# mrafidashti/neuradar

Measured on NVIDIA B200. Metric: train_step_rays_per_sec, higher is better.
Workload: dtype f32

## Files before the change

### neuradar_b200/csrc/common.cuh

```cuda
#pragma once

#include <cuda_runtime.h>
#include <stdint.h>

#include "neuradar_b200.h"

namespace nrb {

constexpr int kWarp = 32;
constexpr unsigned kFull = 0xffffffffu;

void set_error(const char* fmt, ...);
void count_launch();
int finish_launch(const char* what);

inline bool aligned16(const void* p) { return (reinterpret_cast<uintptr_t>(p) & 15u) == 0; }

#define NRB_REQUIRE(cond, code, ...) \
  do {                               \
    if (!(cond)) {                   \
      ::nrb::set_error(__VA_ARGS__); \
      return (code);                 \
    }                                \
  } while (0)

int check_grid(const nrb_grid_t* g);
int check_rays(const nrb_rays_t* r);
int check_intervals(const char* who, const nrb_intervals_t* iv);

inline unsigned blocks_for(int64_t work, int threads) { return static_cast<unsigned>((work + threads - 1) / threads); }
int sm_count();
cudaError_t ensure_dynamic_smem(const void* kernel, int bytes);

__device__ __forceinline__ float mul(float a, float b) { return __fmul_rn(a, b); }
__device__ __forceinline__ float add(float a, float b) { return __fadd_rn(a, b); }
__device__ __forceinline__ float sub(float a, float b) { return __fsub_rn(a, b); }
__device__ __forceinline__ float div(float a, float b) { return __fdiv_rn(a, b); }

constexpr float kThird = 0.333333343267440796f;

struct Gaussian {
  float x, y, z;
  float std;
};

__device__ __forceinline__ Gaussian contract_gaussian(float mx, float my, float mz, float std, float scale) {
  mx = div(mx, scale);
  my = div(my, scale);
  mz = div(mz, scale);
  std = div(std, scale);
  const float mag = fmaxf(fmaxf(fabsf(mx), fabsf(my)), fabsf(mz));
  if (!(mag < 1.0f)) {
    const float cm = fmaxf(mag, 1.0f);
    const float k = sub(2.0f, div(1.0f, cm));
    mx = mul(k, div(mx, cm));
    my = mul(k, div(my, cm));
    mz = mul(k, div(mz, cm));
    const float r = div(powf(sub(mul(2.0f, cm), 1.0f), kThird), cm);
    std = mul(std, mul(r, r));
  }
  Gaussian g;
  g.x = mul(add(mx, 2.0f), 0.25f);
  g.y = mul(add(my, 2.0f), 0.25f);
  g.z = mul(add(mz, 2.0f), 0.25f);
  g.std = mul(std, 0.25f);
  return g;
}

__device__ __forceinline__ Gaussian world_gaussian(float ox, float oy, float oz, float dx, float dy, float dz,
                                                   float pixel_area, float start, float end) {
  const float dist = mul(sub(end, start), 0.5f);
  const float t = add(start, dist);
  Gaussian g;
  g.x = add(ox, mul(dx, t));
  g.y = add(oy, mul(dy, t));
  g.z = add(oz, mul(dz, t));
  const float area = mul(pixel_area, mul(t, t));
  g.std = powf(mul(area, dist), kThird);
  return g;
}

__device__ __forceinline__ Gaussian sample_gaussian(float ox, float oy, float oz, float dx, float dy, float dz,
                                                    float pixel_area, float start, float end, float scale) {
  const Gaussian w = world_gaussian(ox, oy, oz, dx, dy, dz, pixel_area, start, end);
  return contract_gaussian(w.x, w.y, w.z, w.std, scale);
}

__device__ __forceinline__ float level_weight(float scal, float std) {
  return div(1.0f, fmaxf(mul(mul(scal, 2.0f), std), 1.0f));
}

constexpr uint32_t kPrimeY = 2654435761u;
constexpr uint32_t kPrimeZ = 805459861u;

struct Cell {
  uint32_t row[8];
  float ox, oy, oz;
};

__device__ __forceinline__ Cell locate_cell(float px, float py, float pz, float scal, uint32_t mask) {
  const float sx = mul(px, scal), sy = mul(py, scal), sz = mul(pz, scal);
  const float fx = floorf(sx), fy = floorf(sy), fz = floorf(sz);
  Cell c;
  c.ox = sub(sx, fx);
  c.oy = sub(sy, fy);
  c.oz = sub(sz, fz);
  const uint32_t xf = static_cast<uint32_t>(static_cast<int32_t>(fx));
  const uint32_t xc = static_cast<uint32_t>(static_cast<int32_t>(ceilf(sx)));
  const uint32_t yf = static_cast<uint32_t>(static_cast<int32_t>(fy)) * kPrimeY;
  const uint32_t yc = static_cast<uint32_t>(static_cast<int32_t>(ceilf(sy))) * kPrimeY;
  const uint32_t zf = static_cast<uint32_t>(static_cast<int32_t>(fz)) * kPrimeZ;
  const uint32_t zc = static_cast<uint32_t>(static_cast<int32_t>(ceilf(sz))) * kPrimeZ;
  c.row[0] = (xc ^ yc ^ zc) & mask;
  c.row[1] = (xc ^ yf ^ zc) & mask;
  c.row[2] = (xf ^ yf ^ zc) & mask;
  c.row[3] = (xf ^ yc ^ zc) & mask;
  c.row[4] = (xc ^ yc ^ zf) & mask;
  c.row[5] = (xc ^ yf ^ zf) & mask;
  c.row[6] = (xf ^ yf ^ zf) & mask;
  c.row[7] = (xf ^ yc ^ zf) & mask;
  return c;
}

__device__ __forceinline__ void corner_weights(const Cell& c, float w[8]) {
  const float ax = c.ox, bx = 1.0f - c.ox, ay = c.oy, by = 1.0f - c.oy, az = c.oz, bz = 1.0f - c.oz;
  w[0] = ax * ay * az;
  w[1] = ax * by * az;
  w[2] = bx * by * az;
  w[3] = bx * ay * az;
  w[4] = ax * ay * bz;
  w[5] = ax * by * bz;
  w[6] = bx * by * bz;
  w[7] = bx * ay * bz;
}

template <int F>
struct Feat;
template <>
struct Feat<1> {
  using type = float;
};
template <>
struct Feat<2> {
  using type = float2;
};
template <>
struct Feat<4> {
  using type = float4;
};

template <int F>
__device__ __forceinline__ void load_row(const float* __restrict__ base, uint32_t row, float v[F]) {
  using V = typename Feat<F>::type;
  const V t = __ldg(reinterpret_cast<const V*>(base) + row);
  if constexpr (F == 1) {
    v[0] = t;
  } else if constexpr (F == 2) {
    v[0] = t.x;
    v[1] = t.y;
  } else {
    v[0] = t.x;
    v[1] = t.y;
    v[2] = t.z;
    v[3] = t.w;
  }
}

template <int F>
__device__ __forceinline__ void load_x_pair(const float* __restrict__ base, uint32_t row_f, uint32_t row_c, float vf[F],
                                            float vc[F]) {
  if constexpr (F == 1) {
    if (row_c == (row_f ^ 1u)) {
      const bool f_low = (row_f & 1u) == 0;
      const float2 t = __ldg(reinterpret_cast<const float2*>(base) + (row_f >> 1));
      vf[0] = f_low ? t.x : t.y;
      vc[0] = f_low ? t.y : t.x;
      return;
    }
  }
  load_row<F>(base, row_f, vf);
  load_row<F>(base, row_c, vc);
}

template <int F>
__device__ __forceinline__ void interpolate(const float* __restrict__ level_base, const Cell& c, float out[F]) {
  float f[8][F];
  load_x_pair<F>(level_base, c.row[3], c.row[0], f[3], f[0]);
  load_x_pair<F>(level_base, c.row[2], c.row[1], f[2], f[1]);
  load_x_pair<F>(level_base, c.row[7], c.row[4], f[7], f[4]);
  load_x_pair<F>(level_base, c.row[6], c.row[5], f[6], f[5]);
  const float ax = c.ox, bx = 1.0f - c.ox, ay = c.oy, by = 1.0f - c.oy, az = c.oz, bz = 1.0f - c.oz;
#pragma unroll
  for (int j = 0; j < F; ++j) {
    const float f03 = f[0][j] * ax + f[3][j] * bx;
    const float f12 = f[1][j] * ax + f[2][j] * bx;
    const float f56 = f[5][j] * ax + f[6][j] * bx;
    const float f47 = f[4][j] * ax + f[7][j] * bx;
    const float f0312 = f03 * ay + f12 * by;
    const float f4756 = f47 * ay + f56 * by;
    out[j] = f0312 * az + f4756 * bz;
  }
}

template <int F>
__device__ __forceinline__ float3 position_grad(const float* __restrict__ level_base, const Cell& c, const float (&g)[F]) {
  float f[8][F];
#pragma unroll
  for (int k = 0; k < 8; ++k) load_row<F>(level_base, c.row[k], f[k]);
  const float ax = c.ox, bx = 1.0f - c.ox, ay = c.oy, by = 1.0f - c.oy, az = c.oz, bz = 1.0f - c.oz;
  float gx = 0.f, gy = 0.f, gz = 0.f;
#pragma unroll
  for (int j = 0; j < F; ++j) {
    const float f03 = f[0][j] * ax + f[3][j] * bx, f12 = f[1][j] * ax + f[2][j] * bx;
    const float f56 = f[5][j] * ax + f[6][j] * bx, f47 = f[4][j] * ax + f[7][j] * bx;
    const float f0312 = f03 * ay + f12 * by, f4756 = f47 * ay + f56 * by;
    gz += g[j] * (f0312 - f4756);
    gy += g[j] * ((f03 - f12) * az + (f47 - f56) * bz);
    gx += g[j] * (((f[0][j] - f[3][j]) * ay + (f[1][j] - f[2][j]) * by) * az +
                  ((f[4][j] - f[7][j]) * ay + (f[5][j] - f[6][j]) * by) * bz);
  }
  return make_float3(gx, gy, gz);
}

__device__ __forceinline__ const float* tile_image_chunk(const float* img, int64_t m, int c) {
  return img + ((m >> 7) * 1024 + (m & 127)) * 4 + c * 512;
}

__device__ __forceinline__ float warp_sum(float v) {
#pragma unroll
  for (int o = 16; o > 0; o >>= 1) v += __shfl_xor_sync(kFull, v, o);
  return v;
}

__device__ __forceinline__ float warp_inclusive_sum(float v, int lane) {
#pragma unroll
  for (int o = 1; o < 32; o <<= 1) {
    const float n = __shfl_up_sync(kFull, v, o);
    if (lane >= o) v += n;
  }
  return v;
}

__device__ __forceinline__ double warp_inclusive_sum(double v, int lane) {
#pragma unroll
  for (int o = 1; o < 32; o <<= 1) {
    const double n = __shfl_up_sync(kFull, v, o);
    if (lane >= o) v += n;
  }
  return v;
}

__device__ __forceinline__ float warp_inclusive_prod(float v, int lane) {
#pragma unroll
  for (int o = 1; o < 32; o <<= 1) {
    const float n = __shfl_up_sync(kFull, v, o);
    if (lane >= o) v *= n;
  }
  return v;
}

__device__ __forceinline__ float nan_to_num(float v) {
  if (isnan(v)) return 0.0f;
  if (isinf(v)) return v > 0 ? 3.402823466e+38f : -3.402823466e+38f;
  return v;
}

__device__ __forceinline__ float power_fn(float x, float lam) {
  const float lam1 = fabsf(lam - 1.0f);
  const float base = add(div(x, lam1), 1.0f);
  const float p = (lam == -1.0f) ? div(1.0f, base) : powf(base, lam);
  return mul(div(lam1, lam), sub(p, 1.0f));
}

// ... 14 lines not shown
```

### neuradar_b200/csrc/hash_bwd_plan.cuh

```cuda
#pragma once

#include <algorithm>

#include "common.cuh"

namespace nrb {

struct GridDev {
  const float* table;
  float scalings[NRB_MAX_LEVELS];
  int num_levels;
  int log2_size;
};

inline GridDev to_dev(const nrb_grid_t* g) {
  GridDev d;
  d.table = g->table;
  for (int i = 0; i < NRB_MAX_LEVELS; ++i) d.scalings[i] = g->scalings[i];
  d.num_levels = g->num_levels;
  d.log2_size = g->log2_hashmap_size;
  return d;
}

struct BwdPlan {
  float* scratch;
  int64_t offset[NRB_MAX_LEVELS];
  int64_t stride[NRB_MAX_LEVELS];
  int copies[NRB_MAX_LEVELS];
  int r1[NRB_MAX_LEVELS];
};

template <int F>
__device__ __forceinline__ void scatter_row(float* __restrict__ base, uint32_t row, const float (&v)[F]) {
  float* p = base + static_cast<size_t>(row) * F;
  if constexpr (F == 1) {
    atomicAdd(p, v[0]);
  } else if constexpr (F == 2) {
    atomicAdd(reinterpret_cast<float2*>(p), make_float2(v[0], v[1]));
  } else {
    atomicAdd(reinterpret_cast<float4*>(p), make_float4(v[0], v[1], v[2], v[3]));
  }
}

template <int F>
__device__ __forceinline__ void scatter_x_pair(float* __restrict__ base, uint32_t row_f, uint32_t row_c,
                                               const float (&vf)[F], const float (&vc)[F], bool quad) {
  if (row_c == row_f) {
    float t[F];
#pragma unroll
    for (int j = 0; j < F; ++j) t[j] = vf[j] + vc[j];
    scatter_row<F>(base, row_f, t);
    return;
  }
  if constexpr (F == 1) {
    if (quad && (row_f ^ row_c) < 4u) {
      const uint32_t sf = row_f & 3u, sc = row_c & 3u;
      const float4 t = make_float4(sf == 0 ? vf[0] : (sc == 0 ? vc[0] : 0.0f), sf == 1 ? vf[0] : (sc == 1 ? vc[0] : 0.0f),
                                   sf == 2 ? vf[0] : (sc == 2 ? vc[0] : 0.0f), sf == 3 ? vf[0] : (sc == 3 ? vc[0] : 0.0f));
      atomicAdd(reinterpret_cast<float4*>(base) + (row_f >> 2), t);
      return;
    }
  } else if constexpr (F == 2) {
    if (row_c == (row_f ^ 1u)) {
      const bool f_low = (row_f & 1u) == 0;
      atomicAdd(reinterpret_cast<float4*>(base) + (row_f >> 1), f_low ? make_float4(vf[0], vf[1], vc[0], vc[1])
                                                                     : make_float4(vc[0], vc[1], vf[0], vf[1]));
      return;
    }
  }
  scatter_row<F>(base, row_f, vf);
  scatter_row<F>(base, row_c, vc);
}

template <int F>
__device__ __forceinline__ void scatter_rows8(float* __restrict__ base, const uint32_t (&row)[8], const float (&v)[8][F],
                                              bool quad) {
  scatter_x_pair<F>(base, row[3], row[0], v[3], v[0], quad);
  scatter_x_pair<F>(base, row[2], row[1], v[2], v[1], quad);
  scatter_x_pair<F>(base, row[7], row[4], v[7], v[4], quad);
  scatter_x_pair<F>(base, row[6], row[5], v[6], v[5], quad);
}

template <int F>
__device__ __forceinline__ void scatter_corners(const BwdPlan& plan, int l, int log2_size, int xf, int yf, int zf, int xc,
                                                int yc, int zc, const uint32_t (&hashed_rows)[8], const float (&v)[8][F],
                                                float* __restrict__ dtable, unsigned spread) {
  const int copies = plan.copies[l];
  if (copies > 1) {
    const int R1 = plan.r1[l];
    if (xf >= 0 && yf >= 0 && zf >= 0 && xc < R1 && yc < R1 && zc < R1) {
      float* rep = plan.scratch + plan.offset[l] + static_cast<size_t>(spread % static_cast<unsigned>(copies)) * plan.stride[l];
      const int cx[8] = {xc, xc, xf, xf, xc, xc, xf, xf};
      const int cy[8] = {yc, yf, yf, yc, yc, yf, yf, yc};
      const int cz[8] = {zc, zc, zc, zc, zf, zf, zf, zf};
      uint32_t rows[8];
#pragma unroll
      for (int k = 0; k < 8; ++k) rows[k] = static_cast<uint32_t>((cz[k] * R1 + cy[k]) * R1 + cx[k]);
      scatter_rows8<F>(rep, rows, v, true);
      return;
    }
  }
  scatter_rows8<F>(dtable + (static_cast<size_t>(l) << log2_size) * F, hashed_rows, v, log2_size >= 2);
}

constexpr int kMergeMaxRuns = 26;

template <int F>
__device__ __forceinline__ void merge_runs_and_scatter(const BwdPlan& plan, int l, int log2_size, float px, float py,
                                                       float pz, float scal, const Cell& c, float (&v)[8][F], bool valid,
                                                       int lane, float* __restrict__ dtable, unsigned spread) {
  const float sx = mul(px, scal), sy = mul(py, scal), sz = mul(pz, scal);
  const int xf = static_cast<int>(floorf(sx)), yf = static_cast<int>(floorf(sy)), zf = static_cast<int>(floorf(sz));
  const int xc = static_cast<int>(ceilf(sx)), yc = static_cast<int>(ceilf(sy)), zc = static_cast<int>(ceilf(sz));
  const int ceq = (xc == xf ? 1 : 0) | (yc == yf ? 2 : 0) | (zc == zf ? 4 : 0) | (valid ? 8 : 0);
  const int pxf = __shfl_up_sync(kFull, xf, 1), pyf = __shfl_up_sync(kFull, yf, 1), pzf = __shfl_up_sync(kFull, zf, 1);
  const int pce = __shfl_up_sync(kFull, ceq, 1);
  const bool head = lane == 0 || pxf != xf || pyf != yf || pzf != zf || pce != ceq;
  const unsigned heads = __ballot_sync(kFull, head);
  bool issue = valid;
  if (__popc(heads) <= kMergeMaxRuns) {
    const unsigned above = heads & ~((2u << lane) - 1u);
    const int next_head = above != 0 ? __ffs(above) - 1 : 32;
#pragma unroll
    for (int d = 1; d < 32; d <<= 1) {
      const bool take = lane + d < next_head;
      if (!__any_sync(kFull, take)) break;
#pragma unroll
      for (int k = 0; k < 8; ++k)
#pragma unroll
        for (int j = 0; j < F; ++j) {
          const float t = __shfl_down_sync(kFull, v[k][j], d);
          if (take) v[k][j] += t;
        }
    }
    issue = valid && head;
  }
  if (issue) scatter_corners<F>(plan, l, log2_size, xf, yf, zf, xc, yc, zc, c.row, v, dtable, spread);
}

inline int64_t plan_hash_bwd(const nrb_grid_t* grid, int64_t M, BwdPlan* plan) {
  constexpr double kMaxBytesPerLevel = 32.0 * 1024 * 1024;
  const int F = grid->features_per_level;
  const double table_rows = static_cast<double>(int64_t{1} << grid->log2_hashmap_size);
  int64_t floats = 0;
  for (int l = 0; l < NRB_MAX_LEVELS; ++l) {
    plan->copies[l] = 0;
    plan->offset[l] = 0;
    plan->stride[l] = 0;
    plan->r1[l] = 0;
    if (l >= grid->num_levels || M < (int64_t{1} << 16)) continue;
    const int64_t r1 = static_cast<int64_t>(grid->scalings[l]) + 1;
    const double verts = static_cast<double>(r1) * r1 * r1;
    if (verts * 1.5 > table_rows || r1 > 1024) continue;
    const int64_t per_copy = (r1 * r1 * r1 * F + 3) & ~int64_t{3};
    int copies = std::min(static_cast<int>(table_rows / verts + 0.5), 1024);
    while (copies > 1 && static_cast<double>(copies) * per_copy * 4 > kMaxBytesPerLevel) --copies;
    if (copies <= 1) continue;
    plan->copies[l] = copies;
    plan->stride[l] = per_copy;
    plan->offset[l] = floats;
    plan->r1[l] = static_cast<int>(r1);
    floats += static_cast<int64_t>(copies) * per_copy;
    floats = (floats + 3) & ~int64_t{3};
  }
  return floats * 4;
}

inline int prepare_bwd_plan(const nrb_grid_t* grid, int64_t M, void* workspace, int64_t workspace_bytes, cudaStream_t s,
                            BwdPlan* plan, int64_t* vertices) {
  const int64_t need = plan_hash_bwd(grid, M, plan);
  *vertices = 0;
  if (need > 0 && workspace != nullptr && workspace_bytes >= need && aligned16(workspace)) {
    plan->scratch = static_cast<float*>(workspace);
    cudaError_t e = cudaMemsetAsync(workspace, 0, static_cast<size_t>(need), s);
    NRB_REQUIRE(e == cudaSuccess, static_cast<int>(e), "backward workspace memset failed: %s", cudaGetErrorString(e));
    for (int l = 0; l < grid->num_levels; ++l)
      if (plan->copies[l] > 1) *vertices += static_cast<int64_t>(plan->r1[l]) * plan->r1[l] * plan->r1[l];
  } else {
    plan->scratch = nullptr;
    for (int l = 0; l < NRB_MAX_LEVELS; ++l) plan->copies[l] = 0;
  }
  return NRB_OK;
}

void launch_fold(const nrb_grid_t* grid, const BwdPlan& plan, float* dtable, int64_t vertices, cudaStream_t s);

}
```

### neuradar_b200/csrc/hash_grid.cu

```cuda
#include <algorithm>
#include <cstdlib>

#include "common.cuh"
#include "hash_bwd_plan.cuh"

namespace nrb {

template <int F>
__global__ void __launch_bounds__(256) hash_fwd_kernel(const __grid_constant__ GridDev g, const float* __restrict__ x,
                                                       const float* __restrict__ std, float* __restrict__ out,
                                                       int64_t total) {
  const int64_t gid = static_cast<int64_t>(blockIdx.x) * blockDim.x + threadIdx.x;
  if (gid >= total) return;
  const int64_t m = gid / g.num_levels;
  const int l = static_cast<int>(gid - m * g.num_levels);
  const float scal = g.scalings[l];
  const Cell c = locate_cell(__ldg(x + 3 * m), __ldg(x + 3 * m + 1), __ldg(x + 3 * m + 2), scal,
                             (1u << g.log2_size) - 1u);
  const float* base = g.table + (static_cast<size_t>(l) << g.log2_size) * F;
  float v[F];
  interpolate<F>(base, c, v);
  if (std != nullptr) {
    const float w = level_weight(scal, __ldg(std + m));
#pragma unroll
    for (int j = 0; j < F; ++j) v[j] *= w;
  }
  using V = typename Feat<F>::type;
  V o;
  if constexpr (F == 1) {
    o = v[0];
  } else if constexpr (F == 2) {
    o = make_float2(v[0], v[1]);
  } else {
    o = make_float4(v[0], v[1], v[2], v[3]);
  }
  reinterpret_cast<V*>(out)[gid] = o;
}

constexpr int kFwdWarps = 8;

template <int F>
__global__ void __launch_bounds__(kFwdWarps * 32) hash_fwd_rows_kernel(const __grid_constant__ GridDev g,
                                                                      const float* __restrict__ x,
                                                                      const float* __restrict__ std,
                                                                      float* __restrict__ out, int64_t M) {
  extern __shared__ __align__(16) char fwd_smem[];
  const int warp = threadIdx.x >> 5, lane = threadIdx.x & 31;
  const int L = g.num_levels, RW = L * F, CPR = RW / 4;
  char* tile = fwd_smem + warp * (32 * RW * 4);
  const int64_t base = (static_cast<int64_t>(blockIdx.x) * kFwdWarps + warp) * 32;
  if (base >= M) return;
  const int64_t mc = min(base + lane, M - 1);
  const float px = __ldg(x + 3 * mc), py = __ldg(x + 3 * mc + 1), pz = __ldg(x + 3 * mc + 2);
  const float sd = std != nullptr ? __ldg(std + mc) : 0.0f;
  const uint32_t mask = (1u << g.log2_size) - 1u;
  char* rowp = tile + lane * (RW * 4);
  for (int l = 0; l < L; ++l) {
    const float scal = g.scalings[l];
    const Cell c = locate_cell(px, py, pz, scal, mask);
    float v[F];
    interpolate<F>(g.table + (static_cast<size_t>(l) << g.log2_size) * F, c, v);
    if (std != nullptr) {
      const float w = level_weight(scal, sd);
#pragma unroll
      for (int j = 0; j < F; ++j) v[j] *= w;
    }
    const int f0 = l * F;
    char* dst = rowp + (((f0 >> 2) ^ (lane % CPR)) << 4) + (f0 & 3) * 4;
    if constexpr (F == 4) {
      *reinterpret_cast<float4*>(dst) = make_float4(v[0], v[1], v[2], v[3]);
    } else if constexpr (F == 2) {
      *reinterpret_cast<float2*>(dst) = make_float2(v[0], v[1]);
    } else {
      *reinterpret_cast<float*>(dst) = v[0];
    }
  }
  __syncwarp();
  for (int e = lane; e < 32 * CPR; e += 32) {
    const int r = e / CPR, cc = e - r * CPR;
    if (base + r < M)
      reinterpret_cast<float4*>(out + (base + r) * RW)[cc] =
          *reinterpret_cast<const float4*>(tile + r * (RW * 4) + ((cc ^ (r % CPR)) << 4));
  }
}

__global__ void __launch_bounds__(256) hash_indices_kernel(const __grid_constant__ GridDev g, const float* __restrict__ x,
                                                           int64_t* __restrict__ idx, int64_t total) {
  const int64_t gid = static_cast<int64_t>(blockIdx.x) * blockDim.x + threadIdx.x;
  if (gid >= total) return;
  const int64_t m = gid / g.num_levels;
  const int l = static_cast<int>(gid - m * g.num_levels);
  const Cell c = locate_cell(x[3 * m], x[3 * m + 1], x[3 * m + 2], g.scalings[l], (1u << g.log2_size) - 1u);
  const int64_t off = static_cast<int64_t>(l) << g.log2_size;
#pragma unroll
  for (int k = 0; k < 8; ++k) idx[gid * 8 + k] = off + c.row[k];
}

template <int F, bool kNeedDx>
__global__ void __launch_bounds__(256) hash_bwd_kernel(const __grid_constant__ GridDev g,
                                                       const __grid_constant__ BwdPlan plan,
                                                       const float* __restrict__ x, const float* __restrict__ std,
                                                       const float* __restrict__ dy, float* __restrict__ dtable,
                                                       float* __restrict__ dx, int64_t total) {
  const int64_t gid = static_cast<int64_t>(blockIdx.x) * blockDim.x + threadIdx.x;
  if (gid >= total) return;
  const int64_t m = gid / g.num_levels;
  const int l = static_cast<int>(gid - m * g.num_levels);
  const float scal = g.scalings[l];
  const float px = __ldg(x + 3 * m), py = __ldg(x + 3 * m + 1), pz = __ldg(x + 3 * m + 2);
  const Cell c = locate_cell(px, py, pz, scal, (1u << g.log2_size) - 1u);
  float gr[F];
  load_row<F>(dy + gid * F, 0, gr);
  if (std != nullptr) {
    const float lw = level_weight(scal, __ldg(std + m));
#pragma unroll
    for (int j = 0; j < F; ++j) gr[j] *= lw;
  }
  if constexpr (kNeedDx) {
    const float3 d = position_grad<F>(g.table + (static_cast<size_t>(l) << g.log2_size) * F, c, gr);
    atomicAdd(dx + 3 * m + 0, d.x * scal);
    atomicAdd(dx + 3 * m + 1, d.y * scal);
    atomicAdd(dx + 3 * m + 2, d.z * scal);
  }
  float w[8];
  corner_weights(c, w);
  float v[8][F];
#pragma unroll
  for (int k = 0; k < 8; ++k)
#pragma unroll
    for (int j = 0; j < F; ++j) v[k][j] = w[k] * gr[j];
  const float sx = mul(px, scal), sy = mul(py, scal), sz = mul(pz, scal);
  const int xf = static_cast<int>(floorf(sx)), yf = static_cast<int>(floorf(sy)), zf = static_cast<int>(floorf(sz));
  const int xc = static_cast<int>(ceilf(sx)), yc = static_cast<int>(ceilf(sy)), zc = static_cast<int>(ceilf(sz));
  scatter_corners<F>(plan, l, g.log2_size, xf, yf, zf, xc, yc, zc, c.row, v, dtable, static_cast<unsigned>(gid >> 5));
}

constexpr int kMergeWarps = 8;

template <int F, bool kImage>
__global__ void __launch_bounds__(kMergeWarps * 32) hash_bwd_merge_kernel(const __grid_constant__ GridDev g,
                                                                          const __grid_constant__ BwdPlan plan,
                                                                          const float* __restrict__ x,
                                                                          const float* __restrict__ std,
                                                                          const float* __restrict__ dy,
                                                                          const int32_t* __restrict__ actor_grid_id,
                                                                          float* __restrict__ dtable, int64_t M) {
  extern __shared__ __align__(16) char dy_smem[];
  const int warp = threadIdx.x >> 5, lane = threadIdx.x & 31;
  const int L = g.num_levels, RW = L * F;
  const int CPR = RW / 4;
  char* tile = dy_smem + warp * (32 * RW * 4);
  const int64_t base = (static_cast<int64_t>(blockIdx.x) * kMergeWarps + warp) * 32;
  if (base >= M) return;
  const int64_t m = base + lane;
  const int64_t mc = m < M ? m : (M - 1);
  const bool valid = m < M && (!kImage || actor_grid_id == nullptr || __ldg(actor_grid_id + mc) < 0);
  if constexpr (!kImage) {
    for (int e = lane; e < 32 * CPR; e += 32) {
      const int r = e / CPR, cc = e - r * CPR;
      const int64_t rr = min(base + r, M - 1);
      const float4 t = __ldg(reinterpret_cast<const float4*>(dy + rr * RW) + cc);
      *reinterpret_cast<float4*>(tile + r * (RW * 4) + ((cc ^ (r % CPR)) << 4)) = t;
    }
  }
  const float px = __ldg(x + 3 * mc), py = __ldg(x + 3 * mc + 1), pz = __ldg(x + 3 * mc + 2);
  const float sd = std != nullptr ? __ldg(std + mc) : 0.0f;
  if constexpr (!kImage) __syncwarp();
  const uint32_t mask = (1u << g.log2_size) - 1u;
  const unsigned spread = static_cast<unsigned>(base >> 5);
  for (int l = 0; l < L; ++l) {
    const float scal = g.scalings[l];
    const Cell c = locate_cell(px, py, pz, scal, mask);
    const int f0 = l * F;
    float gr[F];
    if constexpr (kImage) {
      load_row<F>(tile_image_chunk(dy, m, f0 >> 2) + (f0 & 3), 0, gr);
    } else {
      const char* p = tile + lane * (RW * 4) + (((f0 >> 2) ^ (lane % CPR)) << 4) + (f0 & 3) * 4;
      if constexpr (F == 4) {
        const float4 t = *reinterpret_cast<const float4*>(p);
        gr[0] = t.x, gr[1] = t.y, gr[2] = t.z, gr[3] = t.w;
      } else if constexpr (F == 2) {
        const float2 t = *reinterpret_cast<const float2*>(p);
        gr[0] = t.x, gr[1] = t.y;
      } else {
        gr[0] = *reinterpret_cast<const float*>(p);
      }
    }
    const float lw = (std != nullptr ? level_weight(scal, sd) : 1.0f) * (valid ? 1.0f : 0.0f);
    float w[8];
    corner_weights(c, w);
    float v[8][F];
#pragma unroll
    for (int k = 0; k < 8; ++k)
#pragma unroll
      for (int j = 0; j < F; ++j) v[k][j] = w[k] * (gr[j] * lw);
    merge_runs_and_scatter<F>(plan, l, g.log2_size, px, py, pz, scal, c, v, valid, lane, dtable, spread);
  }
}

template <int F>
__global__ void __launch_bounds__(256) hash_bwd_fold_kernel(const __grid_constant__ GridDev g,
                                                            const __grid_constant__ BwdPlan plan,
                                                            float* __restrict__ dtable, int64_t total_vertices) {
  int64_t v = static_cast<int64_t>(blockIdx.x) * blockDim.x + threadIdx.x;
  if (v >= total_vertices) return;
  int l = 0;
  for (; l < g.num_levels; ++l) {
    if (plan.copies[l] <= 1) continue;
    const int64_t nvl = static_cast<int64_t>(plan.r1[l]) * plan.r1[l] * plan.r1[l];
    if (v < nvl) break;
    v -= nvl;
  }
  if (l >= g.num_levels) return;
  const float* rep = plan.scratch + plan.offset[l] + v * F;
  float sum[F];
#pragma unroll
  for (int j = 0; j < F; ++j) sum[j] = 0.0f;
  for (int cpy = 0; cpy < plan.copies[l]; ++cpy) {
    float t[F];
    load_row<F>(rep + static_cast<size_t>(cpy) * plan.stride[l], 0, t);
#pragma unroll
    for (int j = 0; j < F; ++j) sum[j] += t[j];
  }
  bool any = false;
#pragma unroll
  for (int j = 0; j < F; ++j) any |= (sum[j] != 0.0f);
  if (!any) return;
  const int R1 = plan.r1[l];
  const int ix = static_cast<int>(v % R1), iy = static_cast<int>((v / R1) % R1), iz = static_cast<int>(v / (R1 * R1));
  const uint32_t row = (static_cast<uint32_t>(ix) ^ (static_cast<uint32_t>(iy) * kPrimeY) ^
                        (static_cast<uint32_t>(iz) * kPrimeZ)) & ((1u << g.log2_size) - 1u);
  scatter_row<F>(dtable + (static_cast<size_t>(l) << g.log2_size) * F, row, sum);
}

void launch_fold(const nrb_grid_t* grid, const BwdPlan& plan, float* dtable, int64_t vertices, cudaStream_t s) {
  if (vertices <= 0) return;
  count_launch();
  const unsigned blocks = blocks_for(vertices, 256);
  switch (grid->features_per_level) {
    case 1: hash_bwd_fold_kernel<1><<<blocks, 256, 0, s>>>(to_dev(grid), plan, dtable, vertices); break;
    case 2: hash_bwd_fold_kernel<2><<<blocks, 256, 0, s>>>(to_dev(grid), plan, dtable, vertices); break;
    default: hash_bwd_fold_kernel<4><<<blocks, 256, 0, s>>>(to_dev(grid), plan, dtable, vertices); break;
  }
}

__global__ void __launch_bounds__(256) frustum_gaussians_kernel(const float* __restrict__ origins,
                                                                const float* __restrict__ directions,
                                                                const float* __restrict__ pixel_area,
                                                                nrb_intervals_t iv, float scale,
                                                                float* __restrict__ x, float* __restrict__ std,
                                                                int64_t total) {
  const int64_t gid = static_cast<int64_t>(blockIdx.x) * blockDim.x + threadIdx.x;
  if (gid >= total) return;
  const int S = iv.num_samples;
  const int64_t n = gid / S;
  const int s = static_cast<int>(gid - n * S);
  const Gaussian g = sample_gaussian(origins[3 * n], origins[3 * n + 1], origins[3 * n + 2], directions[3 * n],
                                     directions[3 * n + 1], directions[3 * n + 2], pixel_area[n],
                                     iv.starts[n * iv.row_stride + s], iv.ends[n * iv.row_stride + s], scale);
  x[3 * gid + 0] = g.x;
  x[3 * gid + 1] = g.y;
  x[3 * gid + 2] = g.z;
  std[gid] = g.std;
}

}

using namespace nrb;

extern "C" int nrb_hash_fwd(const nrb_grid_t* grid, const float* x, const float* std, float* out, int64_t M,
                            nrb_stream_t stream) {
  if (int rc = check_grid(grid)) return rc;
  NRB_REQUIRE(x && out && M >= 0, NRB_ERR_BAD_ARG, "nrb_hash_fwd: null pointer or negative M");
  NRB_REQUIRE(aligned16(out), NRB_ERR_ALIGNMENT, "nrb_hash_fwd: out must be 16-byte aligned");
  if (M == 0) return NRB_OK;
  const int64_t total = M * grid->num_levels;
  const GridDev g = to_dev(grid);
  auto s = static_cast<cudaStream_t>(stream);
  const unsigned blocks = blocks_for(total, 256);
  const int row_floats = grid->num_levels * grid->features_per_level;
  if (row_floats >= 4 && row_floats <= 64 && (row_floats & (row_floats - 1)) == 0 && M >= 32) {
    const size_t smem = static_cast<size_t>(kFwdWarps) * 32 * row_floats * 4;
    const unsigned nb = blocks_for(M, kFwdWarps * 32);
#define NRB_ROWS(F)                                                                                                    \
  {                                                                                                                    \
    cudaError_t e = ensure_dynamic_smem(reinterpret_cast<const void*>(hash_fwd_rows_kernel<F>), 64 * 1024); \
    NRB_REQUIRE(e == cudaSuccess, static_cast<int>(e), "nrb_hash_fwd: cudaFuncSetAttribute: %s", cudaGetErrorString(e)); \
    hash_fwd_rows_kernel<F><<<nb, kFwdWarps * 32, smem, s>>>(g, x, std, out, M);                                        \
  }
    switch (grid->features_per_level) {
      case 1: NRB_ROWS(1) break;
      case 2: NRB_ROWS(2) break;
      default: NRB_ROWS(4) break;
    }
#undef NRB_ROWS
    return finish_launch("nrb_hash_fwd");
  }
  switch (grid->features_per_level) {
    case 1: hash_fwd_kernel<1><<<blocks, 256, 0, s>>>(g, x, std, out, total); break;
    case 2: hash_fwd_kernel<2><<<blocks, 256, 0, s>>>(g, x, std, out, total); break;
    default: hash_fwd_kernel<4><<<blocks, 256, 0, s>>>(g, x, std, out, total); break;
  }
  return finish_launch("nrb_hash_fwd");
}

extern "C" int nrb_hash_indices(const nrb_grid_t* grid, const float* x, int64_t* idx, int64_t M,
                                nrb_stream_t stream) {
  if (int rc = check_grid(grid)) return rc;
  NRB_REQUIRE(x && idx && M >= 0, NRB_ERR_BAD_ARG, "nrb_hash_indices: null pointer or negative M");
  if (M == 0) return NRB_OK;
  const int64_t total = M * grid->num_levels;
  hash_indices_kernel<<<blocks_for(total, 256), 256, 0, static_cast<cudaStream_t>(stream)>>>(to_dev(grid), x, idx,
                                                                                             total);
  return finish_launch("nrb_hash_indices");
}

extern "C" int64_t nrb_hash_bwd_workspace_bytes(const nrb_grid_t* grid, int64_t M) {
  if (grid == nullptr || check_grid(grid) != NRB_OK) return -1;
  BwdPlan plan;
  return plan_hash_bwd(grid, M, &plan);
}

template <int F>
static int launch_hash_bwd(const nrb_grid_t* grid, const GridDev& g, const float* x, const float* std, const float* dy,
                           float* dtable, float* dx, int64_t M, void* workspace, int64_t workspace_bytes,
                           cudaStream_t s) {
  BwdPlan plan;
  int64_t vertices = 0;
  if (int rc = prepare_bwd_plan(grid, M, workspace, workspace_bytes, s, &plan, &vertices)) return rc;
  const int64_t total = M * grid->num_levels;
  const unsigned blocks = blocks_for(total, 256);
  const int row_floats = grid->num_levels * F;
  if (dx == nullptr && row_floats >= 4 && row_floats <= 64 && (row_floats & (row_floats - 1)) == 0 && M >= 32) {
    const size_t smem = static_cast<size_t>(kMergeWarps) * 32 * row_floats * 4;
    cudaError_t e = ensure_dynamic_smem(reinterpret_cast<const void*>(hash_bwd_merge_kernel<F, false>), 64 * 1024);
    NRB_REQUIRE(e == cudaSuccess, static_cast<int>(e), "nrb_hash_bwd: cudaFuncSetAttribute: %s", cudaGetErrorString(e));
    hash_bwd_merge_kernel<F, false><<<blocks_for(M, kMergeWarps * 32), kMergeWarps * 32, smem, s>>>(g, plan, x, std, dy,
                                                                                                    nullptr, dtable, M);
  } else if (dx != nullptr) {
    hash_bwd_kernel<F, true><<<blocks, 256, 0, s>>>(g, plan, x, std, dy, dtable, dx, total);
  } else {
    hash_bwd_kernel<F, false><<<blocks, 256, 0, s>>>(g, plan, x, std, dy, dtable, dx, total);
  }
  launch_fold(grid, plan, dtable, vertices, s);
  return finish_launch("nrb_hash_bwd");
}

extern "C" int nrb_hash_bwd(const nrb_grid_t* grid, const float* x, const float* std, const float* dy, float* dtable,
                            float* dx, int64_t M, void* workspace, int64_t workspace_bytes, nrb_stream_t stream) {
// ... 59 lines not shown
```

### neuradar_b200/csrc/proposal_fused.cu

```cuda
#include "actor_grid.cuh"
#include "common.cuh"
#include "hash_bwd_plan.cuh"

namespace nrb {

constexpr int kPropWarps = 4;
constexpr int kMaxChunks = NRB_MAX_SAMPLES / 32;

struct PropGrid {
  const float* table;
  float scalings[NRB_MAX_LEVELS];
  const float* decoder;
  int num_levels;
  int log2_size;
  const int32_t* agid;
  const float* apos;
  const float* astd;
  ActorGridsDev ag;
  float* adtables[NRB_MAX_ACTORS];
};

template <int F, bool kSave>
__global__ void __launch_bounds__(kPropWarps * 32) proposal_fwd_kernel(
    const __grid_constant__ PropGrid g, const float* __restrict__ origins, const float* __restrict__ directions,
// ... 62 lines not shown
        }
      }
      dens = expf(pre);
      if constexpr (kSave) saved_pre[n * S + i] = pre;
      if (density != nullptr) density[n * S + i] = dens;
      dd = mul(sub(end, start), dens);
    }
    const float incl = warp_inclusive_sum(dd, lane);
    float excl = __shfl_up_sync(kFull, incl, 1);
    if (lane == 0) excl = 0.0f;
    const float alpha = 1.0f - expf(-dd);
    const float trans = expf(-(carry + excl));
    if (ok) weights[n * S + i] = nan_to_num(alpha * trans);
    carry += __shfl_sync(kFull, incl, 31);
  }
}

template <int F, int kChunks>
__global__ void __launch_bounds__(kPropWarps * 32) proposal_bwd_kernel(
    const __grid_constant__ PropGrid g, const __grid_constant__ BwdPlan plan, const float* __restrict__ origins, const float* __restrict__ directions,
    const float* __restrict__ pixel_area, float scale, nrb_intervals_t iv, int64_t N, int rays_per_block,
    const float* __restrict__ saved_feats, const float* __restrict__ saved_pre, const float* __restrict__ dweights,
    const float* __restrict__ ddensity, float* __restrict__ dtable, float* __restrict__ ddecoder) {
  extern __shared__ float s_gpre[];
  __shared__ float s_ddec[NRB_MAX_LEVELS * 4];
  __shared__ float s_dec[NRB_MAX_LEVELS * 4];
  const int lane = threadIdx.x & 31;
  const int warp = threadIdx.x >> 5;
  const int S = iv.num_samples;
  const int LF = g.num_levels * F;
  if (threadIdx.x < NRB_MAX_LEVELS * 4) {
    s_ddec[threadIdx.x] = 0.0f;
    s_dec[threadIdx.x] = threadIdx.x < LF ? g.decoder[threadIdx.x] : 0.0f;
  }
  const int64_t n0 = static_cast<int64_t>(blockIdx.x) * rays_per_block;
  const int rays = static_cast<int>(min(static_cast<int64_t>(rays_per_block), N - n0));
#pragma unroll 1
  for (int r = warp; r < rays; r += kPropWarps) {
    const int64_t n = n0 + r;
    const float* st = iv.starts + n * iv.row_stride;
    const float* en = iv.ends + n * iv.row_stride;
    float delta[kChunks], dd[kChunks], trans[kChunks], pre[kChunks];
    float carry = 0.0f;
#pragma unroll
    for (int c = 0; c < kChunks; ++c) {
      if (c * 32 < S) {
        const int i = c * 32 + lane;
        const bool ok = i < S;
        pre[c] = ok ? saved_pre[n * S + i] : 0.0f;
        delta[c] = ok ? sub(en[i], st[i]) : 0.0f;
        dd[c] = ok ? mul(delta[c], expf(pre[c])) : 0.0f;
        const float incl = warp_inclusive_sum(dd[c], lane);
        float excl = __shfl_up_sync(kFull, incl, 1);
        if (lane == 0) excl = 0.0f;
        trans[c] = expf(-(carry + excl));
        carry += __shfl_sync(kFull, incl, 31);
      }
    }
    float suffix = 0.0f;
#pragma unroll
    for (int c = kChunks - 1; c >= 0; --c) {
      if (c * 32 < S) {
        const int i = c * 32 + lane;
        const bool ok = i < S;
        const float e = expf(-dd[c]);
        const float w = (1.0f - e) * trans[c];
        float gwt = (ok && dweights != nullptr) ? dweights[n * S + i] : 0.0f;
        if (isnan(w) || isinf(w)) gwt = 0.0f;
        const float gw = ok ? gwt * w : 0.0f;
        float incl = gw;
#pragma unroll
        for (int o = 1; o < 32; o <<= 1) {
          const float v = __shfl_down_sync(kFull, incl, o);
          if (lane + o < 32) incl += v;
        }
        float excl = __shfl_down_sync(kFull, incl, 1);
        if (lane == 31) excl = 0.0f;
        const float later = suffix + excl;
        if (ok) {
          float gdens = (gwt * trans[c] * e - later) * delta[c];
          if (ddensity != nullptr) gdens += ddensity[n * S + i];
          s_gpre[r * S + i] = gdens * expf(fminf(fmaxf(pre[c], -15.0f), 15.0f));
        }
        suffix += __shfl_sync(kFull, incl, 0);
      }
    }
  }
  __syncthreads();
  const int total = rays * S;
  const int chunks = (total + 31) >> 5;
  const int per_warp = (chunks + kPropWarps - 1) / kPropWarps;
  const int c_end = min(chunks, (warp + 1) * per_warp);
  const unsigned spread = static_cast<unsigned>(blockIdx.x * kPropWarps + warp);
  const uint32_t mask = (1u << g.log2_size) - 1u;
#pragma unroll 1
  for (int c = warp * per_warp; c < c_end; ++c) {
    const int k = c * 32 + lane;
    const bool act = k < total;
    const int kc = act ? k : total - 1;
    const int r = kc / S;
    const int i = kc - r * S;
    const int64_t n = n0 + r;
    const int64_t m = n0 * S + kc;
    const float gpre = act ? s_gpre[kc] : 0.0f;
    const Gaussian q = sample_gaussian(origins[3 * n], origins[3 * n + 1], origins[3 * n + 2], directions[3 * n],
                                       directions[3 * n + 1], directions[3 * n + 2], pixel_area[n],
                                       iv.starts[n * iv.row_stride + i], iv.ends[n * iv.row_stride + i], scale);
    const float* sf = saved_feats + m * LF;
    const int agid = g.agid != nullptr ? g.agid[m] : -1;
    if (act && agid >= 0) {
      const float ax = g.apos[3 * m], ay = g.apos[3 * m + 1], az = g.apos[3 * m + 2];
      const float asd = g.astd[m];
      const uint32_t amask = (1u << g.ag.log2_size) - 1u;
#pragma unroll
      for (int l = 0; l < kActorLevels; ++l) {
        const float scal = g.ag.scalings[l];
        const Cell cell = locate_cell(ax, ay, az, scal, amask);
        const float lw = level_weight(scal, asd);
        float gr[F];
#pragma unroll
        for (int j = 0; j < F; ++j) gr[j] = gpre * s_dec[l * F + j] * lw;
        float w8[8];
        corner_weights(cell, w8);
        float* dt = g.adtables[agid] + (static_cast<size_t>(l) << g.ag.log2_size) * F;
#pragma unroll
        for (int k8 = 0; k8 < 8; ++k8) {
          float v[F];
#pragma unroll
          for (int j = 0; j < F; ++j) v[j] = gr[j] * w8[k8];
          scatter_row<F>(dt, cell.row[k8], v);
        }
      }
    }
    const bool act_static = act && agid < 0;
#pragma unroll 1
    for (int l = 0; l < g.num_levels; ++l) {
      const float scal = g.scalings[l];
      const Cell cell = locate_cell(q.x, q.y, q.z, scal, mask);
      const float lw = level_weight(scal, q.std);
      float gr[F];
#pragma unroll
      for (int j = 0; j < F; ++j) {
        const float dd_lj = warp_sum(gpre * sf[l * F + j]);
        if (lane == 0) atomicAdd(&s_ddec[l * F + j], dd_lj);
        gr[j] = gpre * s_dec[l * F + j] * lw;
      }
      float w8[8];
      corner_weights(cell, w8);
      float v[8][F];
#pragma unroll
      for (int k8 = 0; k8 < 8; ++k8)
#pragma unroll
        for (int j = 0; j < F; ++j) v[k8][j] = w8[k8] * gr[j];
      merge_runs_and_scatter<F>(plan, l, g.log2_size, q.x, q.y, q.z, scal, cell, v, act_static, lane, dtable, spread);
    }
  }
  __syncthreads();
  if (threadIdx.x < LF && ddecoder != nullptr) atomicAdd(ddecoder + threadIdx.x, s_ddec[threadIdx.x]);
}

static PropGrid make_prop_grid(const nrb_grid_t* grid, const float* decoder, const nrb_actor_grids_t* agrids = nullptr,
                               const nrb_actor_samples_t* asamples = nullptr, float* const* adtables = nullptr) {
  PropGrid out{};
  if (agrids != nullptr) {
    out.ag = to_dev(agrids);
    out.agid = asamples->grid_id, out.apos = asamples->pos, out.astd = asamples->std;
    for (int i = 0; i < agrids->num_grids; ++i) out.adtables[i] = adtables != nullptr ? adtables[i] : nullptr;
  }
  out.table = grid->table;
  for (int i = 0; i < NRB_MAX_LEVELS; ++i) out.scalings[i] = grid->scalings[i];
  out.decoder = decoder;
  out.num_levels = grid->num_levels;
  out.log2_size = grid->log2_hashmap_size;
  return out;
}

static int check_proposal(const char* who, const nrb_rays_t* rays, const nrb_grid_t* grid, const float* decoder_w,
                          float scale, const nrb_intervals_t* iv) {
  if (int rc = check_rays(rays)) return rc;
  if (int rc = check_grid(grid)) return rc;
  if (int rc = check_intervals(who, iv)) return rc;
  NRB_REQUIRE(decoder_w != nullptr, NRB_ERR_BAD_ARG, "%s: null pointer", who);
  NRB_REQUIRE(scale > 0.f, NRB_ERR_BAD_ARG, "%s: static_scale must be positive", who);
  return NRB_OK;
}

}

using namespace nrb;

static int check_prop_actors(const char* who, const nrb_grid_t* grid, const nrb_actor_grids_t* agrids,
                             const nrb_actor_samples_t* asamples) {
  if (agrids == nullptr) return NRB_OK;
  NRB_REQUIRE(agrids->num_grids >= 1 && agrids->num_grids <= NRB_MAX_ACTORS && agrids->num_levels == kActorLevels &&
                  agrids->features_per_level == grid->features_per_level && grid->num_levels >= kActorLevels,
              NRB_ERR_UNSUPPORTED, "%s: actor grids must have 4 levels and the static grid's features per level", who);
  NRB_REQUIRE(asamples && asamples->grid_id && asamples->pos && asamples->std, NRB_ERR_BAD_ARG, "%s: actor samples missing", who);
  for (int i = 0; i < agrids->num_grids; ++i) NRB_REQUIRE(agrids->tables[i] != nullptr, NRB_ERR_BAD_ARG, "%s: actor table %d", who, i);
  return NRB_OK;
}

extern "C" int nrb_proposal_fwd(const nrb_rays_t* rays, const nrb_grid_t* grid, const float* decoder_w,
                                float static_scale, const nrb_intervals_t* iv, float* density, float* weights,
                                float* saved_feats, float* saved_pre, const nrb_actor_grids_t* actor_grids,
                                const nrb_actor_samples_t* actor_samples, nrb_stream_t stream) {
  if (int rc = check_proposal("nrb_proposal_fwd", rays, grid, decoder_w, static_scale, iv)) return rc;
  if (int rc = check_prop_actors("nrb_proposal_fwd", grid, actor_grids, actor_samples)) return rc;
  NRB_REQUIRE(weights != nullptr, NRB_ERR_BAD_ARG, "nrb_proposal_fwd: weights is null");
  NRB_REQUIRE((saved_feats == nullptr) == (saved_pre == nullptr), NRB_ERR_BAD_ARG,
              "nrb_proposal_fwd: saved_feats and saved_pre must be given together");
  const int64_t N = rays->num_rays;
  if (N == 0) return NRB_OK;
  const PropGrid g = make_prop_grid(grid, decoder_w, actor_grids, actor_samples);
  const unsigned blocks = blocks_for(N, kPropWarps);
  auto s = static_cast<cudaStream_t>(stream);
  const bool save = saved_feats != nullptr;
#define NRB_LAUNCH(F, SAVE)                                                                                          \
  proposal_fwd_kernel<F, SAVE><<<blocks, kPropWarps * 32, 0, s>>>(g, rays->origins, rays->directions,               \
                                                                  rays->pixel_area, static_scale, *iv, N,           \
                                                                  density, weights, saved_feats, saved_pre)
  switch (grid->features_per_level) {
    case 1: if (save) NRB_LAUNCH(1, true); else NRB_LAUNCH(1, false); break;
    case 2: if (save) NRB_LAUNCH(2, true); else NRB_LAUNCH(2, false); break;
    default: if (save) NRB_LAUNCH(4, true); else NRB_LAUNCH(4, false); break;
  }
#undef NRB_LAUNCH
  return finish_launch("nrb_proposal_fwd");
}

extern "C" int nrb_proposal_bwd(const nrb_rays_t* rays, const nrb_grid_t* grid, const float* decoder_w,
                                float static_scale, const nrb_intervals_t* iv, const float* saved_feats,
                                const float* saved_pre, const float* dweights, const float* ddensity, float* dtable,
                                float* ddecoder_w, void* workspace, int64_t workspace_bytes,
                                const nrb_actor_grids_t* actor_grids, const nrb_actor_samples_t* actor_samples,
                                float* const* actor_dtables, nrb_stream_t stream) {
  if (int rc = check_proposal("nrb_proposal_bwd", rays, grid, decoder_w, static_scale, iv)) return rc;
  if (int rc = check_prop_actors("nrb_proposal_bwd", grid, actor_grids, actor_samples)) return rc;
  NRB_REQUIRE(actor_grids == nullptr || actor_dtables != nullptr, NRB_ERR_BAD_ARG, "nrb_proposal_bwd: actor gradient tables missing");
  NRB_REQUIRE(saved_feats && saved_pre && dtable, NRB_ERR_BAD_ARG, "nrb_proposal_bwd: null pointer");
  NRB_REQUIRE(dweights || ddensity, NRB_ERR_BAD_ARG, "nrb_proposal_bwd: no upstream gradient");
  NRB_REQUIRE(aligned16(dtable), NRB_ERR_ALIGNMENT, "nrb_proposal_bwd: dtable must be 16-byte aligned");
  const int64_t N = rays->num_rays;
  if (N == 0) return NRB_OK;
  const PropGrid g = make_prop_grid(grid, decoder_w, actor_grids, actor_samples, actor_dtables);
  int rays_per_block = kPropWarps;
  while (rays_per_block < 4 * kPropWarps && (rays_per_block * iv->num_samples) % (kPropWarps * 32) != 0) rays_per_block *= 2;
  if ((rays_per_block * iv->num_samples) % (kPropWarps * 32) != 0) rays_per_block = kPropWarps;
  const unsigned blocks = blocks_for(N, rays_per_block);
  const size_t smem = static_cast<size_t>(rays_per_block) * iv->num_samples * sizeof(float);
  auto s = static_cast<cudaStream_t>(stream);
  BwdPlan plan;
  int64_t vertices = 0;
  if (int rc = prepare_bwd_plan(grid, N * iv->num_samples, workspace, workspace_bytes, s, &plan, &vertices)) return rc;
#define NRB_LAUNCH_C(F, CH)                                                                                          \
  proposal_bwd_kernel<F, CH><<<blocks, kPropWarps * 32, smem, s>>>(g, plan, rays->origins, rays->directions,         \
                                                                   rays->pixel_area, static_scale, *iv, N,           \
                                                                   rays_per_block, saved_feats, saved_pre, dweights, \
                                                                   ddensity, dtable, ddecoder_w)
#define NRB_LAUNCH(F)                                   \
  if (iv->num_samples <= 64) {                          \
    NRB_LAUNCH_C(F, 2);                                 \
  } else if (iv->num_samples <= 128) {                  \
    NRB_LAUNCH_C(F, 4);                                 \
  } else {                                              \
    NRB_LAUNCH_C(F, kMaxChunks);                        \
  }
  switch (grid->features_per_level) {
    case 1: NRB_LAUNCH(1); break;
    case 2: NRB_LAUNCH(2); break;
    default: NRB_LAUNCH(4); break;
  }
#undef NRB_LAUNCH
#undef NRB_LAUNCH_C
  launch_fold(grid, plan, dtable, vertices, s);
  return finish_launch("nrb_proposal_bwd");
}
```

Measured before the change: 15.64 million.

## Use shared-memory segmented reduction for long runs in hash backward merge

Result: no change. 15.75 million (median of 6 runs) (+0.7%).

```diff
diff --git a/neuradar_b200/csrc/common.cuh b/neuradar_b200/csrc/common.cuh
--- a/neuradar_b200/csrc/common.cuh
+++ b/neuradar_b200/csrc/common.cuh
@@ -98,6 +98,24 @@
   float ox, oy, oz;
 };
 
+__device__ __forceinline__ void cell_rows(int ixf, int iyf, int izf, int ixc, int iyc, int izc, uint32_t mask,
+                                          uint32_t (&row)[8]) {
+  const uint32_t xf = static_cast<uint32_t>(ixf);
+  const uint32_t xc = static_cast<uint32_t>(ixc);
+  const uint32_t yf = static_cast<uint32_t>(iyf) * kPrimeY;
+  const uint32_t yc = static_cast<uint32_t>(iyc) * kPrimeY;
+  const uint32_t zf = static_cast<uint32_t>(izf) * kPrimeZ;
+  const uint32_t zc = static_cast<uint32_t>(izc) * kPrimeZ;
+  row[0] = (xc ^ yc ^ zc) & mask;
+  row[1] = (xc ^ yf ^ zc) & mask;
+  row[2] = (xf ^ yf ^ zc) & mask;
+  row[3] = (xf ^ yc ^ zc) & mask;
+  row[4] = (xc ^ yc ^ zf) & mask;
+  row[5] = (xc ^ yf ^ zf) & mask;
+  row[6] = (xf ^ yf ^ zf) & mask;
+  row[7] = (xf ^ yc ^ zf) & mask;
+}
+
 __device__ __forceinline__ Cell locate_cell(float px, float py, float pz, float scal, uint32_t mask) {
   const float sx = mul(px, scal), sy = mul(py, scal), sz = mul(pz, scal);
   const float fx = floorf(sx), fy = floorf(sy), fz = floorf(sz);
@@ -105,20 +123,8 @@
   c.ox = sub(sx, fx);
   c.oy = sub(sy, fy);
   c.oz = sub(sz, fz);
-  const uint32_t xf = static_cast<uint32_t>(static_cast<int32_t>(fx));
-  const uint32_t xc = static_cast<uint32_t>(static_cast<int32_t>(ceilf(sx)));
-  const uint32_t yf = static_cast<uint32_t>(static_cast<int32_t>(fy)) * kPrimeY;
-  const uint32_t yc = static_cast<uint32_t>(static_cast<int32_t>(ceilf(sy))) * kPrimeY;
-  const uint32_t zf = static_cast<uint32_t>(static_cast<int32_t>(fz)) * kPrimeZ;
-  const uint32_t zc = static_cast<uint32_t>(static_cast<int32_t>(ceilf(sz))) * kPrimeZ;
-  c.row[0] = (xc ^ yc ^ zc) & mask;
-  c.row[1] = (xc ^ yf ^ zc) & mask;
-  c.row[2] = (xf ^ yf ^ zc) & mask;
-  c.row[3] = (xf ^ yc ^ zc) & mask;
-  c.row[4] = (xc ^ yc ^ zf) & mask;
-  c.row[5] = (xc ^ yf ^ zf) & mask;
-  c.row[6] = (xf ^ yf ^ zf) & mask;
-  c.row[7] = (xf ^ yc ^ zf) & mask;
+  cell_rows(static_cast<int32_t>(fx), static_cast<int32_t>(fy), static_cast<int32_t>(fz), static_cast<int32_t>(ceilf(sx)),
+            static_cast<int32_t>(ceilf(sy)), static_cast<int32_t>(ceilf(sz)), mask, c.row);
   return c;
 }
 
diff --git a/neuradar_b200/csrc/hash_bwd_plan.cuh b/neuradar_b200/csrc/hash_bwd_plan.cuh
--- a/neuradar_b200/csrc/hash_bwd_plan.cuh
+++ b/neuradar_b200/csrc/hash_bwd_plan.cuh
@@ -106,9 +106,19 @@
 constexpr int kMergeMaxRuns = 26;
 
 template <int F>
+struct MergeScratch {
+  static constexpr int kVals = 8 * F;
+  static constexpr int kRow = kVals + 4;
+  static constexpr int kFloats = 32 * kRow + (32 / kVals - 1) * kVals;
+  __device__ static constexpr int row(int r) { return r * kRow + (r / kVals) * kVals; }
+};
+
+template <int F, bool kSharedMerge>
 __device__ __forceinline__ void merge_runs_and_scatter(const BwdPlan& plan, int l, int log2_size, float px, float py,
-                                                       float pz, float scal, const Cell& c, float (&v)[8][F], bool valid,
-                                                       int lane, float* __restrict__ dtable, unsigned spread) {
+                                                       float pz, float scal, float (&v)[8][F], bool valid,
+                                                       int lane, float* __restrict__ wbuf, float* __restrict__ dtable,
+                                                       unsigned spread) {
+  using MS = MergeScratch<F>;
   const float sx = mul(px, scal), sy = mul(py, scal), sz = mul(pz, scal);
   const int xf = static_cast<int>(floorf(sx)), yf = static_cast<int>(floorf(sy)), zf = static_cast<int>(floorf(sz));
   const int xc = static_cast<int>(ceilf(sx)), yc = static_cast<int>(ceilf(sy)), zc = static_cast<int>(ceilf(sz));
@@ -121,21 +131,82 @@
   if (__popc(heads) <= kMergeMaxRuns) {
     const unsigned above = heads & ~((2u << lane) - 1u);
     const int next_head = above != 0 ? __ffs(above) - 1 : 32;
-#pragma unroll
-    for (int d = 1; d < 32; d <<= 1) {
-      const bool take = lane + d < next_head;
-      if (!__any_sync(kFull, take)) break;
-#pragma unroll
-      for (int k = 0; k < 8; ++k)
-#pragma unroll
-        for (int j = 0; j < F; ++j) {
-          const float t = __shfl_down_sync(kFull, v[k][j], d);
-          if (take) v[k][j] += t;
-        }
-    }
     issue = valid && head;
-  }
-  if (issue) scatter_corners<F>(plan, l, log2_size, xf, yf, zf, xc, yc, zc, c.row, v, dtable, spread);
+    const bool short_runs = (heads | (heads << 1) | (heads << 2) | (heads << 3)) == ~0u;
+    if (!kSharedMerge || short_runs) {
+#pragma unroll
+      for (int d = 1; d < (kSharedMerge ? 4 : 32); d <<= 1) {
+        const bool take = lane + d < next_head;
+        if (!__any_sync(kFull, take)) break;
+#pragma unroll
+        for (int k = 0; k < 8; ++k)
+#pragma unroll
+          for (int j = 0; j < F; ++j) {
+            const float t = __shfl_down_sync(kFull, v[k][j], d);
+            if (take) v[k][j] += t;
+          }
+      }
+    } else if constexpr (kSharedMerge) {
+      constexpr int K = MS::kVals;
+      float* own = wbuf + MS::row(lane);
+#pragma unroll
+      for (int q = 0; q < K / 4; ++q) {
+        const int e = q * 4;
+        *reinterpret_cast<float4*>(own + e) = make_float4(v[e / F][e % F], v[(e + 1) / F][(e + 1) % F],
+                                                          v[(e + 2) / F][(e + 2) % F], v[(e + 3) / F][(e + 3) % F]);
+      }
+      __syncwarp();
+      const int idx = lane % K, s0 = lane - idx;
+      float* col = wbuf + MS::row(s0) + idx;
+      const unsigned hs = heads >> s0;
+      float acc = col[0];
+#pragma unroll
+      for (int t = 1; t < K; ++t) {
+        const float x = col[t * MS::kRow];
+        if ((hs >> t) & 1u) {
+          col[(t - 1) * MS::kRow] = acc;
+          acc = x;
+        } else {
+          acc += x;
+        }
+      }
+      col[(K - 1) * MS::kRow] = acc;
+      if constexpr (K < 32) {
+        const unsigned below = heads & ((1u << s0) - 1u);
+        const int hsl = s0 > 0 ? (31 - __clz(below)) / K : 0;
+        float carry = 0.0f;
+#pragma unroll
+        for (int k = 1; k < 32 / K; ++k) {
+          const float t = __shfl_up_sync(kFull, acc, k * K);
+          if (s0 / K - k >= hsl) carry += t;
+        }
+        if ((hs & 1u) == 0) {
+          const unsigned inner = hs & ((1u << K) - 2u);
+          const int end = inner != 0 ? __ffs(inner) - 2 : K - 1;
+          col[end * MS::kRow] += carry;
+        }
+      }
+      __syncwarp();
+      if (issue) {
+        const float* sum = wbuf + MS::row(next_head - 1);
+#pragma unroll
+        for (int q = 0; q < K / 4; ++q) {
+          const int e = q * 4;
+          const float4 t = *reinterpret_cast<const float4*>(sum + e);
+          v[e / F][e % F] = t.x;
+          v[(e + 1) / F][(e + 1) % F] = t.y;
+          v[(e + 2) / F][(e + 2) % F] = t.z;
+          v[(e + 3) / F][(e + 3) % F] = t.w;
+        }
+      }
+      __syncwarp();
+    }
+  }
+  if (issue) {
+    uint32_t rows[8];
+    cell_rows(xf, yf, zf, xc, yc, zc, (1u << log2_size) - 1u, rows);
+    scatter_corners<F>(plan, l, log2_size, xf, yf, zf, xc, yc, zc, rows, v, dtable, spread);
+  }
 }
 
 inline int64_t plan_hash_bwd(const nrb_grid_t* grid, int64_t M, BwdPlan* plan) {
diff --git a/neuradar_b200/csrc/hash_grid.cu b/neuradar_b200/csrc/hash_grid.cu
--- a/neuradar_b200/csrc/hash_grid.cu
+++ b/neuradar_b200/csrc/hash_grid.cu
@@ -138,7 +138,10 @@
 constexpr int kMergeWarps = 8;
 
 template <int F, bool kImage>
-__global__ void __launch_bounds__(kMergeWarps * 32) hash_bwd_merge_kernel(const __grid_constant__ GridDev g,
+constexpr int kMergeMinBlocks = F == 4 ? (kImage ? 4 : 3) : 5;
+
+template <int F, bool kImage>
+__global__ void __launch_bounds__(kMergeWarps * 32, kMergeMinBlocks<F, kImage>) hash_bwd_merge_kernel(const __grid_constant__ GridDev g,
                                                                           const __grid_constant__ BwdPlan plan,
                                                                           const float* __restrict__ x,
                                                                           const float* __restrict__ std,
@@ -146,6 +149,7 @@
                                                                           const int32_t* __restrict__ actor_grid_id,
                                                                           float* __restrict__ dtable, int64_t M) {
   extern __shared__ __align__(16) char dy_smem[];
+  __shared__ __align__(16) float merge_smem[kMergeWarps * MergeScratch<F>::kFloats];
   const int warp = threadIdx.x >> 5, lane = threadIdx.x & 31;
   const int L = g.num_levels, RW = L * F;
   const int CPR = RW / 4;
@@ -195,7 +199,8 @@
     for (int k = 0; k < 8; ++k)
 #pragma unroll
       for (int j = 0; j < F; ++j) v[k][j] = w[k] * (gr[j] * lw);
-    merge_runs_and_scatter<F>(plan, l, g.log2_size, px, py, pz, scal, c, v, valid, lane, dtable, spread);
+    merge_runs_and_scatter<F, true>(plan, l, g.log2_size, px, py, pz, scal, v, valid, lane,
+                                    merge_smem + warp * MergeScratch<F>::kFloats, dtable, spread);
   }
 }
 
diff --git a/neuradar_b200/csrc/proposal_fused.cu b/neuradar_b200/csrc/proposal_fused.cu
--- a/neuradar_b200/csrc/proposal_fused.cu
+++ b/neuradar_b200/csrc/proposal_fused.cu
@@ -238,7 +238,8 @@
       for (int k8 = 0; k8 < 8; ++k8)
 #pragma unroll
         for (int j = 0; j < F; ++j) v[k8][j] = w8[k8] * gr[j];
-      merge_runs_and_scatter<F>(plan, l, g.log2_size, q.x, q.y, q.z, scal, cell, v, act_static, lane, dtable, spread);
+      merge_runs_and_scatter<F, false>(plan, l, g.log2_size, q.x, q.y, q.z, scal, v, act_static, lane, nullptr, dtable,
+                                       spread);
     }
   }
   __syncthreads();
```
